# allentran/golds-rl-gym

Measured on AMD Instinct MI355X. Metric: env-steps/sec (whole node), 32k parallel Swarm-v0 envs, 20-step PAAC rollout, higher is better.
Workload: dtype f32; 1 GPU; Swarm-v0 84x84, 32768 envs per GPU, T=20 PAAC update, conv policy of train_paac_conv.py (BASELINE configs[2]); envs_per_gpu=32768, envs_total=32768, rollout_steps=20, policy=conv, train=True, swarm_math=exact, env_state_dtype=f64, streams=4, gradient_exchange=none

## Files before the change

golds-rl-gym_amd/csrc/api.hip:

```cpp
#include <string.h>

#include <algorithm>
#include <mutex>
#include <set>
#include <cmath>

#include "common.h"
#include "rollout_dev.h"

static thread_local std::string g_create_error;
static std::mutex g_live_mutex;
static std::set<const grl_handle *> g_live_handles;

namespace grl {
bool grl_handle_alive(const grl_handle *h) {
    std::lock_guard<std::mutex> lk(g_live_mutex);
    return g_live_handles.count(h) != 0;
}
void grl_sync_for_destroy(grl_handle *h) {
    if (grl_handle_alive(h)) {
        hipSetDevice(h->cfg.device_id);
        if (h->stream) hipStreamSynchronize(h->stream);
    } else {
        hipDeviceSynchronize();
// ... 47 lines not shown
            case GRL_FLD_RESET_XA: fi = {h->sw.rxa, 8, 20, false}; return h->sw.rxa != nullptr;
            case GRL_FLD_RESET_PNOISE: fi = {h->sw.rpnoise, 8, 160, false}; return h->sw.rpnoise != nullptr;
            case GRL_FLD_RESET_ANOISE: fi = {h->sw.ranoise, 8, 20, false}; return h->sw.ranoise != nullptr;
            default: return false;
        }
    }
    if (kind == GRL_ENV_SOLOW) {
        switch (f) {
            case GRL_FLD_SOLOW_K: fi = {h->so.k, 4, 1, false}; return true;
            case GRL_FLD_SOLOW_Z: fi = {h->so.z, 4, (size_t)h->so.P, true}; return true;
            case GRL_FLD_SOLOW_Z0: fi = {h->so.z0, 4, (size_t)h->so.P, true}; return true;
            case GRL_FLD_SOLOW_E: fi = {h->so.e, 4, (size_t)h->so.Q, true}; return true;
            case GRL_FLD_SOLOW_TAPE: fi = {h->so.tape, 4, (size_t)h->cfg.solow_tape_len, true}; return true;
            case GRL_FLD_SOLOW_TAPE_POS: fi = {h->so.tape_pos, 4, 1, false}; return true;
            case GRL_FLD_NHIST: fi = {h->so.nhist, 4, 1, false}; return true;
            default: return false;
        }
    }
    if (kind == GRL_ENV_TRADE) {
        size_t n = h->cfg.n_assets;
        switch (f) {
            case GRL_FLD_TRADE_CASH: fi = {h->tr.cash, 8, 1, false}; return true;
            case GRL_FLD_TRADE_ASSETS: fi = {h->tr.assets, 8, 1, false}; return true;
            case GRL_FLD_TRADE_QUANTITY: fi = {h->tr.q, 8, n, true}; return true;
            case GRL_FLD_TRADE_PRICES: fi = {h->tr.p, 8, n, true}; return true;
            case GRL_FLD_TRADE_NORMALS: fi = {h->tr.normals, 4, n, true}; return true;
            case GRL_FLD_NHIST: fi = {h->tr.nhist, 4, 1, false}; return true;
            default: return false;
        }
    }
    if (kind == GRL_ENV_TICKER) {
        switch (f) {
            case GRL_FLD_TICKER_CASH: fi = {h->tk.cash, 8, 1, false}; return true;
            case GRL_FLD_TICKER_ASSETS: fi = {h->tk.assets, 8, 1, false}; return true;
            case GRL_FLD_TICKER_QUANTITY: fi = {h->tk.q, 8, 2, false}; return true;
            case GRL_FLD_TICKER_IDX: fi = {h->tk.idx, 4, 1, false}; return true;
            case GRL_FLD_TICKER_START: fi = {h->tk.start, 4, 1, false}; return true;
            case GRL_FLD_TICKER_START0: fi = {h->tk.start0, 4, 1, false}; return true;
            case GRL_FLD_NHIST: fi = {h->tk.nhist, 4, 1, false}; return true;
            default: return false;
        }
    }
    return false;
}

static int action_cols(const grl_handle *h) {
    switch (h->cfg.env_kind) {
        case GRL_ENV_SWARM: return N_AGENTS * 2;
        case GRL_ENV_SOLOW: return 1;
        case GRL_ENV_TICKER: return 4;
        default: return h->cfg.n_assets;
    }
}

__global__ void episodes_account_kernel(const float *__restrict__ reward, const uint8_t *__restrict__ done, int env_base, int E,
                                        double *__restrict__ total, int32_t *__restrict__ len, int64_t *__restrict__ steps,
                                        grl_episode_record *__restrict__ rec, int32_t *__restrict__ count, int cap) {
    const int e = env_base + blockIdx.x * blockDim.x + threadIdx.x;
    const bool active = e < E;
    episodes_account_env(active, e, active ? reward[e] : 0.f, active && done[e] != 0, total, len, steps, rec, count, cap);
}

int episodes_launch_account(grl_handle *h, int env_base, int count) {
    if (!h->ep_total) return GRL_OK;
    if (count < 0) count = h->E - env_base;
    hipLaunchKernelGGL(episodes_account_kernel, dim3((count + 255) / 256), dim3(256), 0, h->stream, h->reward, h->done, env_base,
                       env_base + count, h->ep_total, h->ep_len, h->ep_steps, h->ep_rec, h->ep_count, h->ep_capacity);
    GRL_HIP(h, hipGetLastError());
    return GRL_OK;
}

static int reset_list(grl_handle *h, const int32_t *list_dev, const int32_t *count_dev, int max_count) {
    switch (h->cfg.env_kind) {
        case GRL_ENV_SWARM: return swarm_launch_reset(h, list_dev, count_dev, max_count);
        case GRL_ENV_SOLOW: return solow_launch_reset(h, list_dev, count_dev, max_count, true);
        case GRL_ENV_TICKER: return ticker_launch_reset(h, list_dev, count_dev, max_count);
        default: return trade_launch_reset(h, list_dev, count_dev, max_count);
    }
}

}

using namespace grl;

extern "C" {

int grl_abi_version(void) { return GRL_ABI_VERSION; }

int grl_config_default(int32_t env_kind, grl_config *cfg) {
    if (!cfg || env_kind < 0 || env_kind > GRL_ENV_TICKER) return GRL_E_INVALID;
    memset(cfg, 0, sizeof(*cfg));
    cfg->struct_size = (int32_t)sizeof(grl_config);
    cfg->env_kind = env_kind;
    cfg->num_envs = 32;
    cfg->max_episode_steps = env_kind == GRL_ENV_SWARM ? 128 : 1024;
    if (env_kind == GRL_ENV_TICKER) cfg->max_episode_steps = 1023;
    cfg->grid_size = 84;
    cfg->n_assets = 2;
    cfg->solow_p = 1; cfg->solow_q = 1;
    cfg->solow_tape_len = 2048;
    cfg->rnn_length = 5;
    cfg->seed = 1692;
    cfg->solow_sigma = 0.1; cfg->solow_delta = 0.02;
    cfg->trade_std_p = 0.05;
    cfg->trade_starting_balance = 10.0;
    return GRL_OK;
}

int grl_create(const grl_config *cfg, grl_handle **out) {
    if (!cfg || !out) return fail(nullptr, GRL_E_INVALID, "grl_create: null argument");
    *out = nullptr;
    if (cfg->struct_size != (int32_t)sizeof(grl_config)) return fail(nullptr, GRL_E_INVALID, "grl_create: grl_config size mismatch (ABI drift)");
    if (cfg->env_kind < 0 || cfg->env_kind > GRL_ENV_TICKER) return fail(nullptr, GRL_E_INVALID, "grl_create: unknown env_kind");
    if (cfg->env_kind == GRL_ENV_TICKER && (cfg->n_assets != 2 || cfg->rnn_length < 1 || cfg->rnn_length > 32))
        return fail(nullptr, GRL_E_INVALID, "grl_create: the Ticker table has two price columns (n_assets must be 2) and rnn_length must be in 1..32");
    if (cfg->env_kind == GRL_ENV_TICKER && (cfg->max_episode_steps < 0 || cfg->max_episode_steps > 1023))
        return fail(nullptr, GRL_E_INVALID, "grl_create: Ticker episodes live inside a 1024-row window: max_episode_steps must be in 0..1023 (0: no cap, stepping past the window is an error as in the reference)");
    if (cfg->num_envs <= 0) return fail(nullptr, GRL_E_INVALID, "grl_create: num_envs must be positive");
    if (cfg->env_kind == GRL_ENV_SWARM && (cfg->grid_size < 2 || cfg->grid_size > 254)) return fail(nullptr, GRL_E_INVALID, "grl_create: grid_size must be in 2..254");
    if (cfg->env_kind == GRL_ENV_TRADE && (cfg->n_assets < 1 || cfg->n_assets > 64)) return fail(nullptr, GRL_E_INVALID, "grl_create: n_assets must be in 1..64");
    if (cfg->env_kind == GRL_ENV_TRADE && !(cfg->trade_starting_balance > 0.0 && cfg->trade_starting_balance < 1e300))
        return fail(nullptr, GRL_E_INVALID, "grl_create: trade_starting_balance must be a positive finite number (the observation takes log(cash + 1e-4))");
    if (cfg->env_kind == GRL_ENV_SOLOW) {
        if (cfg->solow_p < 1 || cfg->solow_p > 8) return fail(nullptr, GRL_E_INVALID, "grl_create: solow_p must be in 1..8 (p=0 cannot reset in the reference either: fed_env.py:250 indexes an empty z)");
        if (cfg->solow_q < 0 || cfg->solow_q > 8) return fail(nullptr, GRL_E_INVALID, "grl_create: solow_q must be in 0..8");
        if (cfg->solow_tape_len < 2 || (cfg->solow_tape_len & 1)) return fail(nullptr, GRL_E_INVALID, "grl_create: solow_tape_len must be even and >= 2");
        if (cfg->rnn_length < 1 || cfg->rnn_length > 16) return fail(nullptr, GRL_E_INVALID, "grl_create: rnn_length must be in 1..16");
    }
    if (cfg->env_kind == GRL_ENV_TRADE && (cfg->rnn_length < 1 || cfg->rnn_length > 32))
        return fail(nullptr, GRL_E_INVALID, "grl_create: rnn_length must be in 1..32");
    int ndev = 0;
    hipError_t e = hipGetDeviceCount(&ndev);
    if (e != hipSuccess || ndev <= 0)
        return fail(nullptr, GRL_E_NO_DEVICE, std::string("grl_create: no HIP device available (") + (e != hipSuccess ? hipGetErrorString(e) : "count=0") + "); this library has no CPU path");
    if (cfg->device_id < 0 || cfg->device_id >= ndev) return fail(nullptr, GRL_E_NO_DEVICE, "grl_create: device_id out of range");
    hipDeviceProp_t prop;
    if ((e = hipGetDeviceProperties(&prop, cfg->device_id)) != hipSuccess) return fail(nullptr, GRL_E_HIP, std::string("hipGetDeviceProperties: ") + hipGetErrorString(e));
    if (strncmp(prop.gcnArchName, "gfx950", 6) != 0)
        return fail(nullptr, GRL_E_NO_DEVICE, std::string("grl_create: device is ") + prop.gcnArchName + ", this library is built for gfx950 (MI355X) only");
    if ((e = hipSetDevice(cfg->device_id)) != hipSuccess) return fail(nullptr, GRL_E_HIP, std::string("hipSetDevice: ") + hipGetErrorString(e));

    grl_handle *h = new grl_handle();
    {
        std::lock_guard<std::mutex> lk(g_live_mutex);
        g_live_handles.insert(h);
    }
    h->cfg = *cfg;
    h->E = cfg->num_envs;
    h->step_in_flight = false;
    h->prof_on = false; h->prof_used = 0;
    h->ep_total = nullptr; h->ep_len = nullptr; h->ep_steps = nullptr; h->ep_rec = nullptr; h->ep_count = nullptr; h->ep_capacity = 0;
    h->stream = nullptr; h->ev0 = nullptr; h->ev1 = nullptr;
    h->sw = {}; h->so = {}; h->tr = {}; h->tk = {};
    int rc = GRL_OK;
    auto bail = [&](int code) {
        g_create_error = h->err;
        grl_destroy(h);
        return code;
    };
    if ((e = hipStreamCreateWithFlags(&h->stream, hipStreamNonBlocking)) != hipSuccess) return bail(hip_fail(h, e, "hipStreamCreate"));
    if ((e = hipEventCreate(&h->ev0)) != hipSuccess || (e = hipEventCreate(&h->ev1)) != hipSuccess) return bail(hip_fail(h, e, "hipEventCreate"));
    size_t E = h->E;
    auto dm = [&](void **p, size_t bytes) -> int {
        hipError_t ee = hipMalloc(p, bytes);
        if (ee != hipSuccess) return hip_fail(h, ee, "hipMalloc");
        h->allocs.push_back(*p);
        ee = hipMemsetAsync(*p, 0, bytes, h->stream);
        return ee == hipSuccess ? GRL_OK : hip_fail(h, ee, "hipMemsetAsync");
    };
    h->actions_elems = E * action_cols(h);
    if ((rc = dm((void **)&h->elapsed, E * 4)) || (rc = dm((void **)&h->episode, E * 4)) || (rc = dm((void **)&h->reward, E * 4)) ||
        (rc = dm((void **)&h->done, E)) || (rc = dm((void **)&h->done_list, E * 4)) || (rc = dm((void **)&h->done_count, 16 * 4)) ||
        (rc = dm((void **)&h->err_flag, 4)) || (rc = dm((void **)&h->actions, h->actions_elems * 4)))
        return bail(rc);
    switch (cfg->env_kind) {
        case GRL_ENV_SWARM: rc = swarm_alloc(h); break;
        case GRL_ENV_SOLOW: rc = solow_alloc(h); break;
        case GRL_ENV_TICKER: rc = ticker_alloc(h); break;
        default: rc = trade_alloc(h); break;
    }
    if (rc) return bail(rc);
    if ((e = hipStreamSynchronize(h->stream)) != hipSuccess) return bail(hip_fail(h, e, "hipStreamSynchronize"));
    *out = h;
    return GRL_OK;
}

int grl_destroy(grl_handle *h) {
    if (!h) return GRL_OK;
    hipSetDevice(h->cfg.device_id);
    if (h->stream) hipStreamSynchronize(h->stream);
    for (void *p : h->allocs) hipFree(p);
    for (void *p : h->user_allocs) hipFree(p);
    for (hipEvent_t ev : h->prof_ev) hipEventDestroy(ev);
    if (h->ev0) hipEventDestroy(h->ev0);
    if (h->ev1) hipEventDestroy(h->ev1);
    if (h->stream) hipStreamDestroy(h->stream);
    {
        std::lock_guard<std::mutex> lk(g_live_mutex);
        g_live_handles.erase(h);
    }
    delete h;
    return GRL_OK;
}

const char *grl_last_error(const grl_handle *h) { return h ? h->err.c_str() : g_create_error.c_str(); }

int grl_reset(grl_handle *h, const int32_t *env_idx, int32_t n) {
    if (!h) return GRL_E_INVALID;
    hipSetDevice(h->cfg.device_id);
    int32_t cnt;
    if (env_idx == nullptr) {
        cnt = h->E;
        int rc = launch_iota(h, h->done_list, h->E);
        if (rc) return rc;
    } else {
        if (n < 0 || n > h->E) return fail(h, GRL_E_INVALID, "grl_reset: n out of range");
        for (int i = 0; i < n; ++i)
            if (env_idx[i] < 0 || env_idx[i] >= h->E) return fail(h, GRL_E_INVALID, "grl_reset: env index out of range");
        cnt = n;
        GRL_HIP(h, hipMemcpyAsync(h->done_list, env_idx, (size_t)n * 4, hipMemcpyHostToDevice, h->stream));
    }
    GRL_HIP(h, hipMemcpyAsync(h->done_count, &cnt, 4, hipMemcpyHostToDevice, h->stream));
    GRL_HIP(h, hipStreamSynchronize(h->stream));
    if (cnt > 0) {
        int rc = reset_list(h, h->done_list, h->done_count, cnt);
        if (rc) return rc;
    }
    GRL_HIP(h, hipStreamSynchronize(h->stream));
    return GRL_OK;
}

int grl_swarm_reset_injected(grl_handle *h, const double *x0, const double *xa0, const double *random_actions,
                             const double *agent_noise, const double *particle_noise) {
    if (!h || h->cfg.env_kind != GRL_ENV_SWARM) return fail(h, GRL_E_INVALID, "grl_swarm_reset_injected: not a Swarm handle");
    if (!x0 || !xa0 || !random_actions || !agent_noise || !particle_noise) return fail(h, GRL_E_INVALID, "grl_swarm_reset_injected: null argument");
    hipSetDevice(h->cfg.device_id);
    return swarm_reset_injected(h, x0, xa0, random_actions, agent_noise, particle_noise);
}

int grl_ticker_set_table(grl_handle *h, const double *rows, int32_t nrows) {
    if (!h || h->cfg.env_kind != GRL_ENV_TICKER) return fail(h, GRL_E_INVALID, "grl_ticker_set_table: not a Ticker handle");
    if (!rows) return fail(h, GRL_E_INVALID, "grl_ticker_set_table: null argument");
    hipSetDevice(h->cfg.device_id);
    return ticker_set_table(h, rows, nrows);
}

static int copy_field(grl_handle *h, int32_t field, void *host, size_t bytes, bool to_device) {
    if (!h || !host) return fail(h, GRL_E_INVALID, "grl_set/get_state: null argument");
    hipSetDevice(h->cfg.device_id);
    FieldInfo fi;
    if (!field_info(h, field, fi)) return fail(h, GRL_E_INVALID, "grl_set/get_state: field not valid for this env kind/config");
    size_t E = h->E, total = E * fi.inner * fi.elem;
    if (bytes != total) return fail(h, GRL_E_SIZE, "grl_set/get_state: host buffer is " + std::to_string(bytes) + " bytes, field needs " + std::to_string(total));
    GRL_HIP(h, hipStreamSynchronize(h->stream));
    if (!fi.feature_major || fi.inner == 1) {
        if (to_device) GRL_HIP(h, hipMemcpy(fi.dev, host, total, hipMemcpyHostToDevice));
        else GRL_HIP(h, hipMemcpy(host, fi.dev, total, hipMemcpyDeviceToHost));
        return GRL_OK;
    }
    auto transpose = [&](auto *hp, auto &tmp) -> int {
        if (to_device) {
            for (size_t e = 0; e < E; ++e)
                for (size_t i = 0; i < fi.inner; ++i) tmp[i * E + e] = hp[e * fi.inner + i];
            GRL_HIP(h, hipMemcpy(fi.dev, tmp.data(), total, hipMemcpyHostToDevice));
        } else {
            GRL_HIP(h, hipMemcpy(tmp.data(), fi.dev, total, hipMemcpyDeviceToHost));
            for (size_t e = 0; e < E; ++e)
                for (size_t i = 0; i < fi.inner; ++i) hp[e * fi.inner + i] = tmp[i * E + e];
        }
        return GRL_OK;
    };
    if (fi.elem == 8) {
        std::vector<uint64_t> tmp(E * fi.inner);
        return transpose((uint64_t *)host, tmp);
    }
    std::vector<uint32_t> tmp(E * fi.inner);
    return transpose((uint32_t *)host, tmp);
}

int grl_set_state(grl_handle *h, int32_t field, const void *host, size_t bytes) { return copy_field(h, field, (void *)host, bytes, true); }
int grl_get_state(grl_handle *h, int32_t field, void *host, size_t bytes) { return copy_field(h, field, host, bytes, false); }

int grl_step_device(grl_handle *h, const float *actions_dev) {
    if (!h || !actions_dev) return fail(h, GRL_E_INVALID, "grl_step_device: null argument");
    hipSetDevice(h->cfg.device_id);
    int rc;
    switch (h->cfg.env_kind) {
        case GRL_ENV_SWARM: rc = swarm_launch_step(h, actions_dev); break;
        case GRL_ENV_SOLOW: rc = solow_launch_step(h, actions_dev); break;
        case GRL_ENV_TICKER: rc = ticker_launch_step(h, actions_dev); break;
        default: rc = trade_launch_step(h, actions_dev); break;
    }
    if (rc == GRL_OK) rc = episodes_launch_account(h);
    if (rc == GRL_OK) h->step_in_flight = true;
    return rc;
}

int grl_step_async(grl_handle *h, const float *actions_host) {
    if (!h || !actions_host) return fail(h, GRL_E_INVALID, "grl_step_async: null argument");
    hipSetDevice(h->cfg.device_id);
    GRL_HIP(h, hipMemcpyAsync(h->actions, actions_host, h->actions_elems * 4, hipMemcpyHostToDevice, h->stream));
    return grl_step_device(h, h->actions);
}

int grl_swarm_step_f64(grl_handle *h, const double *actions_host) {
    if (!h || !actions_host) return fail(h, GRL_E_INVALID, "grl_swarm_step_f64: null argument");
// ... 369 lines not shown
```

golds-rl-gym_amd/csrc/common.h:

```cpp
#pragma once
#include <hip/hip_runtime.h>
#include <stdint.h>
#include <string>
#include <vector>

#include "../../include/goldsrl.h"

namespace grl {

constexpr int N_LOCUSTS = 80;
constexpr int N_AGENTS = 10;
constexpr int N_POINTS = 90;
constexpr int N_BURN_IN = 10;
constexpr int SWARM_EPB = 4;
constexpr int SWARM_TPB = SWARM_EPB * N_LOCUSTS;

enum : uint32_t {
    RS_SWARM_X0 = 0, RS_SWARM_XA0 = 1, RS_SWARM_RANDACT = 2, RS_SWARM_ANOISE = 3, RS_SWARM_PNOISE = 4,
    RS_SOLOW_Z0 = 8, RS_SOLOW_TAPE = 9, RS_TRADE_PRICE = 12, RS_TICKER_START = 16, RS_USER = 64
};

struct SwarmState {
    double *x, *xa, *pnoise, *anoise;
    double *rx, *rxa, *rpnoise, *ranoise;
    double *reward64;
    double *act64;
    uint8_t *lbins, *abins, *pos;
};

struct SolowState {
    float *k, *z, *e, *z0;
    float *tape;
    int32_t *tape_pos, *nhist;
    float *obs_raw, *obs, *history;
    float rho_z[8], rho_e[8];
    int P, Q;
};

struct TradeState {
    double *cash, *assets, *q, *p;
    float *normals;
    uint32_t *nstep;
    int32_t *nhist;
    float *obs_raw, *obs;
    double std_e;
    double start;
};

struct TickerState {
    double *cash, *assets, *q;
    double *reward64;
    int32_t *idx, *start, *start0;
    int32_t *nhist;
    float *obs_raw, *obs;
    const double *table;
    int rows;
};

}

struct grl_handle {
    grl_config cfg;
    int E;
    hipStream_t stream;
    hipEvent_t ev0, ev1;
    std::string err;
    bool step_in_flight;
    int32_t *elapsed, *episode;
    float *reward;
    uint8_t *done;
    int32_t *done_list, *done_count;
    int32_t *err_flag;
    float *actions;
    size_t actions_elems;
    grl::SwarmState sw;
    grl::SolowState so;
    grl::TradeState tr;
    grl::TickerState tk;
    std::vector<void *> allocs;
    std::vector<void *> user_allocs;
    double *ep_total;
    int32_t *ep_len;
    int64_t *ep_steps;
    grl_episode_record *ep_rec;
    int32_t *ep_count;
    int32_t ep_capacity;
    bool prof_on;
    std::vector<hipEvent_t> prof_ev;
    size_t prof_used;
};

namespace grl {
int fail(grl_handle *h, int code, const std::string &msg);
bool grl_handle_alive(const grl_handle *h);
void grl_sync_for_destroy(grl_handle *h);
void prof_begin(grl_handle *h);
void prof_end(grl_handle *h);
int hip_fail(grl_handle *h, hipError_t e, const char *what);
#define GRL_HIP(h, call)                                        \
    do {                                                        \
        hipError_t _e = (call);                                 \
        if (_e != hipSuccess) return grl::hip_fail(h, _e, #call); \
    } while (0)

int episodes_launch_account(grl_handle *h, int env_base = 0, int count = -1);
int swarm_alloc(grl_handle *h);
int swarm_launch_step(grl_handle *h, const float *actions_dev, const double *actions64_dev = nullptr, int no_wind = 0);
int swarm_launch_step_range(grl_handle *h, const float *actions_dev, int env_base, int count, int slot, bool counter_zeroed = false);
int swarm_launch_reset(grl_handle *h, const int32_t *list_dev, const int32_t *count_dev, int max_count);
int swarm_launch_observe(grl_handle *h);
int swarm_reset_injected(grl_handle *h, const double *x0, const double *xa0, const double *ra,
                         const double *an, const double *pn);
int swarm_materialize(grl_handle *h, int first, int count, float *out_dev);
int solow_alloc(grl_handle *h);
int solow_launch_step(grl_handle *h, const float *actions_dev);
int solow_launch_reset(grl_handle *h, const int32_t *list_dev, const int32_t *count_dev, int max_count, bool advance_episode);
int solow_launch_observe(grl_handle *h);
int trade_alloc(grl_handle *h);
int trade_launch_step(grl_handle *h, const float *actions_dev);
int trade_launch_reset(grl_handle *h, const int32_t *list_dev, const int32_t *count_dev, int max_count);
int trade_launch_observe(grl_handle *h);
int ticker_alloc(grl_handle *h);
int ticker_set_table(grl_handle *h, const double *rows_host, int nrows);
int ticker_launch_step(grl_handle *h, const float *actions_dev);
int ticker_launch_reset(grl_handle *h, const int32_t *list_dev, const int32_t *count_dev, int max_count);
int ticker_launch_observe(grl_handle *h);
int launch_returns(grl_handle *h, const float *r, const float *v, const float *mask, const float *boot, int T, int B,
                   float gamma, float lam, float scale, float clip_lo, float clip_hi, float *y, float *adv);
int launch_transform(grl_handle *h, int kind, float *actions_dev, int rows, int cols);
int launch_randn(grl_handle *h, float *dst, size_t n, uint32_t stream, uint64_t counter);
int launch_iota(grl_handle *h, int32_t *dst, int n);
}
```

golds-rl-gym_amd/csrc/swarm.hip:

```cpp
#include "common.h"
#include "rng.h"

namespace grl {

struct SwarmParams {
    double *x, *xa, *pnoise, *anoise;
    const double *rx, *rxa, *rpn, *ran;
    const double *inj_x0, *inj_xa0, *inj_ra, *inj_an, *inj_pn;
    const float *actions;
    const double *actions64;
    int32_t *elapsed, *episode;
    float *reward;
    double *reward64;
    uint8_t *done, *lbins, *abins, *pos;
    int32_t *done_list, *done_count;
    const int32_t *reset_list, *reset_count;
    int E, grid, max_steps;
    int env_base;
    uint32_t flags, env_off;
    uint64_t seed;
    int no_wind;
};

constexpr int LDS_STRIDE = 97;

struct SwarmLds {
    double2 p[SWARM_EPB][LDS_STRIDE];
    double en[SWARM_EPB][N_LOCUSTS];
    double meanx[SWARM_EPB];
    double rew[SWARM_EPB];
    int dflag[SWARM_EPB];
};

constexpr double DT = 0.05, NOISE = 0.0001, WIND = 1.0, GRAV = -1.0, FATT = 0.5, LATT = 10.0;

__device__ __forceinline__ void cutoff(double &y, double &vx, double &vy) {
    if (y <= 0) {
        y = 0;
        vx = 0;
        if (vy <= 0) vy = 0;
    }
}

__device__ __forceinline__ void x_update(double &x, double &y, double vx, double vy, double nx, double ny) {
    cutoff(y, vx, vy);
    x = x + (DT * vx + NOISE * nx);
    y = y + (DT * vy + NOISE * ny);
    if (y <= 0) y = 0;
}

__device__ __forceinline__ void x_update_f32v(double &x, double &y, float vx, float vy, double nx, double ny) {
    if (y <= 0) {
        y = 0;
        vx = 0;
        if (vy <= 0) vy = 0;
    }
    x = x + ((double)(0.05f * vx) + NOISE * nx);
    y = y + ((double)(0.05f * vy) + NOISE * ny);
    if (y <= 0) y = 0;
}

template <bool FAST>
__device__ __forceinline__ void pair_term(double sx, double sy, double xj, double yj, double &t0, double &t1) {
    double dx = sx - xj, dy = sy - yj;
    double d = sqrt(dx * dx + dy * dy);
    if (FAST) {
        double t = exp(d * -0.1);
        double t2 = t * t, t4 = t2 * t2, t5 = t4 * t, t10 = t5 * t5;
        double w = (FATT * t - t10) / (d + 0.000001);
        t0 = w * dx;
        t1 = w * dy;
    } else {
        double s = FATT * exp(-d / LATT) - exp(-d);
        double den = d + 0.000001;
        t0 = s * dx / den;
        t1 = s * dy / den;
    }
}

template <bool FAST>
__device__ __forceinline__ void locust_velocity(const double2 *src, double xj, double yj, double &vx, double &vy) {
    double a0[8], a1[8];
#pragma unroll
    for (int k = 0; k < 8; ++k) pair_term<FAST>(src[k].x, src[k].y, xj, yj, a0[k], a1[k]);
    for (int i = 8; i < N_LOCUSTS; i += 8) {
#pragma unroll
        for (int k = 0; k < 8; ++k) {
            double t0, t1;
            pair_term<FAST>(src[i + k].x, src[i + k].y, xj, yj, t0, t1);
            a0[k] += t0;
            a1[k] += t1;
        }
    }
    double ll0 = ((a0[0] + a0[1]) + (a0[2] + a0[3])) + ((a0[4] + a0[5]) + (a0[6] + a0[7]));
    double ll1 = ((a1[0] + a1[1]) + (a1[2] + a1[3])) + ((a1[4] + a1[5]) + (a1[6] + a1[7]));
#pragma unroll
    for (int k = 0; k < 8; ++k) pair_term<FAST>(src[N_LOCUSTS + k].x, src[N_LOCUSTS + k].y, xj, yj, a0[k], a1[k]);
    double al0 = ((a0[0] + a0[1]) + (a0[2] + a0[3])) + ((a0[4] + a0[5]) + (a0[6] + a0[7]));
    double al1 = ((a1[0] + a1[1]) + (a1[2] + a1[3])) + ((a1[4] + a1[5]) + (a1[6] + a1[7]));
#pragma unroll
    for (int k = 8; k < N_AGENTS; ++k) {
        double t0, t1;
        pair_term<FAST>(src[N_LOCUSTS + k].x, src[N_LOCUSTS + k].y, xj, yj, t0, t1);
        al0 += t0;
        al1 += t1;
    }
    vx = (WIND + ll0) + al0;
    vy = (GRAV + ll1) + al1;
}

template <bool FAST>
__device__ __forceinline__ void block_step(SwarmLds &L, int tid, int el, int j, double &xj, double &yj, double actx,
                                           double acty, double anx, double any, double pnx, double pny, bool act32 = false,
                                           bool wind = true) {
    if (tid < SWARM_EPB * N_AGENTS) {
        int ea = tid / N_AGENTS, a = tid - ea * N_AGENTS;
        double2 q = L.p[ea][N_LOCUSTS + a];
        if (act32) x_update_f32v(q.x, q.y, wind ? (float)actx + 1.0f : (float)actx, (float)acty, anx, any);
        else x_update(q.x, q.y, wind ? actx + WIND : actx, acty, anx, any);
        L.p[ea][N_LOCUSTS + a] = q;
    }
    L.p[el][j] = make_double2(xj, yj);
    __syncthreads();
    double vx, vy;
    locust_velocity<FAST>(L.p[el], xj, yj, vx, vy);
    L.en[el][j] = vx * vx + vy * vy;
    x_update(xj, yj, vx, vy, pnx, pny);
    __syncthreads();
    L.p[el][j] = make_double2(xj, yj);
    if (j == 0) {
        const double *e = L.en[el];
        double r[8];
#pragma unroll
        for (int k = 0; k < 8; ++k) r[k] = e[k];
        for (int i = 8; i < N_LOCUSTS; i += 8) {
#pragma unroll
            for (int k = 0; k < 8; ++k) r[k] += e[i + k];
        }
        double s = ((r[0] + r[1]) + (r[2] + r[3])) + ((r[4] + r[5]) + (r[6] + r[7]));
        L.rew[el] = -(s / (double)N_LOCUSTS);
    }
    __syncthreads();
}

__device__ __forceinline__ double edge_at(int k, double lo, double hi, double step, int G) {
    return (k >= G) ? hi : ((double)k * step + lo);
}
__device__ __forceinline__ int count_edges_le(double v, double lo, double hi, double step, int G) {
    if (!(v >= lo)) return 0;
    if (v >= hi) return G + 1;
    double gf = floor((v - lo) / step);
    int g = (gf > (double)G) ? G : (int)gf;
    if (g < 0) g = 0;
    for (int it = 0; it < 4 && g < G && edge_at(g + 1, lo, hi, step, G) <= v; ++it) ++g;
    for (int it = 0; it < 4 && g > 0 && edge_at(g, lo, hi, step, G) > v; ++it) --g;
    return g + 1;
}

enum { MODE_STEP = 0, MODE_OBSERVE = 1, MODE_RESET = 2 };

template <int MODE, bool FAST>
__global__ __launch_bounds__(SWARM_TPB, MODE == 0 ? 5 : 1) void swarm_kernel(SwarmParams P) {
    __shared__ SwarmLds L;
    __shared__ int env_of[SWARM_EPB];
    const int tid = threadIdx.x;
    const int el = tid / N_LOCUSTS, j = tid - el * N_LOCUSTS;

    if (MODE == MODE_RESET) {
        int cnt = *P.reset_count;
        if ((int)blockIdx.x * SWARM_EPB >= cnt) return;
        if (tid < SWARM_EPB) {
            int li = blockIdx.x * SWARM_EPB + tid;
            env_of[tid] = li < cnt ? P.reset_list[li] : -1;
        }
    } else {
        if (tid < SWARM_EPB) {
            int e = P.env_base + blockIdx.x * SWARM_EPB + tid;
            env_of[tid] = e < P.E ? e : -1;
        }
    }
    __syncthreads();
    const int env = env_of[el];
    const bool active = env >= 0;
    const int ea = tid / N_AGENTS, a = tid - ea * N_AGENTS;
    const bool agent_lane = tid < SWARM_EPB * N_AGENTS;
    const int aenv = agent_lane ? env_of[ea] : -1;
    const bool aactive = aenv >= 0;

    double xj = 0.5, yj = 0.5;
    if (MODE == MODE_STEP || MODE == MODE_OBSERVE) {
        if (active) {
            double2 q = reinterpret_cast<const double2 *>(P.x)[(size_t)env * N_LOCUSTS + j];
            xj = q.x; yj = q.y;
        }
        if (agent_lane) {
            double2 q = make_double2(0.5, 0.5);
            if (aactive) q = reinterpret_cast<const double2 *>(P.xa)[(size_t)aenv * N_AGENTS + a];
            L.p[ea][N_LOCUSTS + a] = q;
        }
    }

    if (MODE == MODE_STEP) {
        double actx = 0, acty = 0, anx = 0, any = 0, pnx = 0, pny = 0;
        if (active) {
            double2 n = reinterpret_cast<const double2 *>(P.pnoise)[(size_t)env * N_LOCUSTS + j];
            pnx = n.x; pny = n.y;
        }
        if (aactive) {
            if (P.actions64) {
                double2 act = reinterpret_cast<const double2 *>(P.actions64)[(size_t)aenv * N_AGENTS + a];
                actx = act.x; acty = act.y;
            } else {
                float2 act = reinterpret_cast<const float2 *>(P.actions)[(size_t)aenv * N_AGENTS + a];
                actx = (double)act.x; acty = (double)act.y;
            }
            double2 n = reinterpret_cast<const double2 *>(P.anoise)[(size_t)aenv * N_AGENTS + a];
            anx = n.x; any = n.y;
        }
        block_step<FAST>(L, tid, el, j, xj, yj, actx, acty, anx, any, pnx, pny, P.actions64 == nullptr, P.no_wind == 0);
        if (active) reinterpret_cast<double2 *>(P.x)[(size_t)env * N_LOCUSTS + j] = make_double2(xj, yj);
        if (aactive) reinterpret_cast<double2 *>(P.xa)[(size_t)aenv * N_AGENTS + a] = L.p[ea][N_LOCUSTS + a];
        if (active && j == 0) {
            double r = L.rew[el];
            int el_new = P.elapsed[env] + 1;
            bool d = (r >= 0) || (P.max_steps > 0 && el_new >= P.max_steps);
            P.elapsed[env] = el_new;
            P.reward64[env] = r;
            P.reward[env] = (float)r;
            P.done[env] = d ? 1 : 0;
            L.dflag[el] = d ? env : -1;
        } else if (j == 0) {
            L.dflag[el] = -1;
        }
        __syncthreads();
        if (tid == 0) {
            int n = 0;
#pragma unroll
            for (int e = 0; e < SWARM_EPB; ++e) n += L.dflag[e] >= 0 ? 1 : 0;
            if (n) {
                int slot = atomicAdd(P.done_count, n);
#pragma unroll
                for (int e = 0; e < SWARM_EPB; ++e)
                    if (L.dflag[e] >= 0) P.done_list[slot++] = L.dflag[e];
            }
        }
    }

    if (MODE == MODE_RESET) {
        const uint32_t genv = active ? (uint32_t)env + P.env_off : 0u;
        const uint32_t gaenv = aactive ? (uint32_t)aenv + P.env_off : 0u;
        const uint32_t ep = (active && !(P.flags & GRL_F_RESEED_EACH_RESET)) ? (uint32_t)P.episode[env] : 0u;
        const uint32_t aep = (aactive && !(P.flags & GRL_F_RESEED_EACH_RESET)) ? (uint32_t)P.episode[aenv] : 0u;
        double pn10x = 0, pn10y = 0, an10x = 0, an10y = 0;
        if (P.flags & GRL_F_RESET_FROM_SNAPSHOT) {
            if (active) {
                double2 q = reinterpret_cast<const double2 *>(P.rx)[(size_t)env * N_LOCUSTS + j];
                xj = q.x; yj = q.y;
                double2 n = reinterpret_cast<const double2 *>(P.rpn)[(size_t)env * N_LOCUSTS + j];
                pn10x = n.x; pn10y = n.y;
            }
            if (agent_lane) {
                double2 q = make_double2(0.5, 0.5);
                if (aactive) {
                    q = reinterpret_cast<const double2 *>(P.rxa)[(size_t)aenv * N_AGENTS + a];
                    double2 n = reinterpret_cast<const double2 *>(P.ran)[(size_t)aenv * N_AGENTS + a];
                    an10x = n.x; an10y = n.y;
                }
                L.p[ea][N_LOCUSTS + a] = q;
            }
            L.p[el][j] = make_double2(xj, yj);
            __syncthreads();
        } else {
            const bool inj = P.inj_x0 != nullptr;
            if (inj) {
                if (active) {
                    double2 q = reinterpret_cast<const double2 *>(P.inj_x0)[(size_t)env * N_LOCUSTS + j];
                    xj = q.x; yj = q.y;
                }
            } else {
                u01_pair(rng_block(P.seed, genv, ep, RS_SWARM_X0, j), xj, yj);
            }
            if (agent_lane) {
                double2 q = make_double2(0.5, 0.5);
                if (inj) {
                    if (aactive) q = reinterpret_cast<const double2 *>(P.inj_xa0)[(size_t)aenv * N_AGENTS + a];
                } else {
                    u01_pair(rng_block(P.seed, gaenv, aep, RS_SWARM_XA0, a), q.x, q.y);
                }
                L.p[ea][N_LOCUSTS + a] = q;
            }
            for (int t = 0; t <= N_BURN_IN; ++t) {
                double actx = 0, acty = 0, anx = 0, any = 0, pnx = 0, pny = 0;
                if (inj) {
                    if (active) {
                        double2 n = reinterpret_cast<const double2 *>(P.inj_pn)[((size_t)env * (N_BURN_IN + 1) + t) * N_LOCUSTS + j];
                        pnx = n.x; pny = n.y;
                    }
                    if (aactive) {
                        double2 n = reinterpret_cast<const double2 *>(P.inj_an)[((size_t)aenv * (N_BURN_IN + 1) + t) * N_AGENTS + a];
                        anx = n.x; any = n.y;
                        if (t < N_BURN_IN) {
                            double2 r = reinterpret_cast<const double2 *>(P.inj_ra)[((size_t)aenv * N_BURN_IN + t) * N_AGENTS + a];
                            actx = r.x; acty = r.y;
                        }
                    }
                } else {
                    normal_pair(rng_block(P.seed, genv, ep, RS_SWARM_PNOISE, t * N_LOCUSTS + j), pnx, pny);
                    if (agent_lane) {
                        normal_pair(rng_block(P.seed, gaenv, aep, RS_SWARM_ANOISE, t * N_AGENTS + a), anx, any);
                        if (t < N_BURN_IN) normal_pair(rng_block(P.seed, gaenv, aep, RS_SWARM_RANDACT, t * N_AGENTS + a), actx, acty);
                    }
                }
                if (t == N_BURN_IN) {
                    pn10x = pnx; pn10y = pny; an10x = anx; an10y = any;
                    break;
                }
                block_step<FAST>(L, tid, el, j, xj, yj, actx, acty, anx, any, pnx, pny);
            }
        }
        if (active) {
            reinterpret_cast<double2 *>(P.x)[(size_t)env * N_LOCUSTS + j] = make_double2(xj, yj);
            reinterpret_cast<double2 *>(P.pnoise)[(size_t)env * N_LOCUSTS + j] = make_double2(pn10x, pn10y);
            if (j == 0) {
                P.elapsed[env] = 0;
                P.episode[env] = P.episode[env] + 1;
            }
        }
        if (aactive) {
            reinterpret_cast<double2 *>(P.xa)[(size_t)aenv * N_AGENTS + a] = L.p[ea][N_LOCUSTS + a];
            reinterpret_cast<double2 *>(P.anoise)[(size_t)aenv * N_AGENTS + a] = make_double2(an10x, an10y);
        }
    }

    if (MODE == MODE_OBSERVE) {
        L.p[el][j] = make_double2(xj, yj);
        __syncthreads();
    }

    if (P.flags & GRL_F_SWARM_NO_OBSERVE) return;
    if (j == 0) {
        double s = L.p[el][0].x;
        for (int i = 1; i < N_POINTS; ++i) s += L.p[el][i].x;
        L.meanx[el] = s / (double)N_POINTS;
    }
    __syncthreads();
    const int G = P.grid;
    const double ylo = 0.0, yhi = 6.0;
    const double ystep = (yhi - ylo) / (double)G;
    {
        double m = L.meanx[el];
        double lo = m - 1.5, hi = m + 1.5;
        double step = (hi - lo) / (double)G;
        int cx = count_edges_le(xj, lo, hi, step, G);
        int cy = count_edges_le(yj, ylo, yhi, ystep, G);
        int bx = (xj == hi) ? G - 1 : cx - 1;
        int by = (yj == yhi) ? G - 1 : cy - 1;
        bool in = bx >= 0 && bx < G && by >= 0 && by < G;
        if (active) reinterpret_cast<uint16_t *>(P.lbins)[(size_t)env * N_LOCUSTS + j] = in ? (uint16_t)(bx | (by << 8)) : (uint16_t)0xFFFF;
    }
    if (aactive) {
        double2 q = L.p[ea][N_LOCUSTS + a];
        double m = L.meanx[ea];
        double lo = m - 1.5, hi = m + 1.5;
        double step = (hi - lo) / (double)G;
        int cx = count_edges_le(q.x, lo, hi, step, G);
        int cy = count_edges_le(q.y, ylo, yhi, ystep, G);
        int bx = (q.x == hi) ? G - 1 : cx - 1;
        int by = (q.y == yhi) ? G - 1 : cy - 1;
        bool in = bx >= 0 && bx < G && by >= 0 && by < G;
        reinterpret_cast<uint16_t *>(P.abins)[(size_t)aenv * N_AGENTS + a] = in ? (uint16_t)(bx | (by << 8)) : (uint16_t)0xFFFF;
        int px = cx >= G ? G - 1 : cx;
        int py = cy >= G ? G - 1 : cy;
        reinterpret_cast<uint16_t *>(P.pos)[(size_t)aenv * N_AGENTS + a] = (uint16_t)(px | (py << 8));
    }
}

__global__ void swarm_materialize_kernel(const uint8_t *lbins, const uint8_t *abins, const uint8_t *pos, int first, int G,
                                         float *out) {
    extern __shared__ unsigned int cnt[];
    const int env = first + blockIdx.x;
    const int GG = G * G;
    for (int i = threadIdx.x; i < 2 * GG; i += blockDim.x) cnt[i] = 0;
    __syncthreads();
    if (threadIdx.x < N_LOCUSTS) {
        int bx = lbins[((size_t)env * N_LOCUSTS + threadIdx.x) * 2], by = lbins[((size_t)env * N_LOCUSTS + threadIdx.x) * 2 + 1];
        if (bx != 255) atomicAdd(&cnt[bx * G + by], 1u);
    } else if (threadIdx.x < N_POINTS) {
        int a = threadIdx.x - N_LOCUSTS;
        int bx = abins[((size_t)env * N_AGENTS + a) * 2], by = abins[((size_t)env * N_AGENTS + a) * 2 + 1];
        if (bx != 255) atomicAdd(&cnt[GG + bx * G + by], 1u);
    }
    __syncthreads();
    float *o = out + (size_t)blockIdx.x * N_AGENTS * GG * 3;
    for (int a = 0; a < N_AGENTS; ++a) {
        int px = pos[((size_t)env * N_AGENTS + a) * 2], py = pos[((size_t)env * N_AGENTS + a) * 2 + 1];
        int hot = px * G + py;
        for (int i = threadIdx.x; i < GG * 3; i += blockDim.x) {
            int pix = i / 3, c = i - pix * 3;
            float v;
            if (c == 0) v = (float)((double)cnt[pix] / 80.0);
            else if (c == 1) v = (float)((double)cnt[GG + pix] / 10.0);
            else v = (pix == hot) ? 1.0f : 0.0f;
            o[(size_t)a * GG * 3 + i] = v;
        }
    }
}

static SwarmParams make_params(grl_handle *h) {
    SwarmParams P{};
    P.x = h->sw.x; P.xa = h->sw.xa; P.pnoise = h->sw.pnoise; P.anoise = h->sw.anoise;
    P.rx = h->sw.rx; P.rxa = h->sw.rxa; P.rpn = h->sw.rpnoise; P.ran = h->sw.ranoise;
    P.elapsed = h->elapsed; P.episode = h->episode; P.reward = h->reward; P.reward64 = h->sw.reward64;
    P.done = h->done; P.lbins = h->sw.lbins; P.abins = h->sw.abins; P.pos = h->sw.pos;
    P.done_list = h->done_list; P.done_count = h->done_count;
    P.E = h->E; P.grid = h->cfg.grid_size; P.max_steps = h->cfg.max_episode_steps;
    P.flags = h->cfg.flags; P.env_off = (uint32_t)h->cfg.env_id_offset; P.seed = h->cfg.seed;
    return P;
}

template <typename T>
static int dmalloc(grl_handle *h, T **p, size_t n) {
    GRL_HIP(h, hipMalloc((void **)p, n * sizeof(T)));
    h->allocs.push_back(*p);
    GRL_HIP(h, hipMemsetAsync(*p, 0, n * sizeof(T), h->stream));
    return GRL_OK;
}

int swarm_alloc(grl_handle *h) {
    size_t E = h->E;
    int rc;
    if ((rc = dmalloc(h, &h->sw.x, E * N_LOCUSTS * 2))) return rc;
    if ((rc = dmalloc(h, &h->sw.xa, E * N_AGENTS * 2))) return rc;
    if ((rc = dmalloc(h, &h->sw.pnoise, E * N_LOCUSTS * 2))) return rc;
    if ((rc = dmalloc(h, &h->sw.anoise, E * N_AGENTS * 2))) return rc;
    if ((rc = dmalloc(h, &h->sw.reward64, E))) return rc;
    if ((rc = dmalloc(h, &h->sw.lbins, E * N_LOCUSTS * 2))) return rc;
    if ((rc = dmalloc(h, &h->sw.abins, E * N_AGENTS * 2))) return rc;
    if ((rc = dmalloc(h, &h->sw.pos, E * N_AGENTS * 2))) return rc;
    if (h->cfg.flags & GRL_F_RESET_FROM_SNAPSHOT) {
        if ((rc = dmalloc(h, &h->sw.rx, E * N_LOCUSTS * 2))) return rc;
        if ((rc = dmalloc(h, &h->sw.rxa, E * N_AGENTS * 2))) return rc;
        if ((rc = dmalloc(h, &h->sw.rpnoise, E * N_LOCUSTS * 2))) return rc;
        if ((rc = dmalloc(h, &h->sw.ranoise, E * N_AGENTS * 2))) return rc;
    }
    return GRL_OK;
}

static inline int nblocks(int n) { return (n + SWARM_EPB - 1) / SWARM_EPB; }

int swarm_launch_step(grl_handle *h, const float *actions_dev, const double *actions64_dev, int no_wind) {
    SwarmParams P = make_params(h);
    P.actions = actions_dev;
    P.actions64 = actions64_dev;
    P.no_wind = no_wind;
    GRL_HIP(h, hipMemsetAsync(h->done_count, 0, sizeof(int32_t), h->stream));
    prof_begin(h);
    if (h->cfg.flags & GRL_F_SWARM_FAST_MATH)
        hipLaunchKernelGGL((swarm_kernel<MODE_STEP, true>), dim3(nblocks(h->E)), dim3(SWARM_TPB), 0, h->stream, P);
    else
        hipLaunchKernelGGL((swarm_kernel<MODE_STEP, false>), dim3(nblocks(h->E)), dim3(SWARM_TPB), 0, h->stream, P);
    prof_end(h);
    GRL_HIP(h, hipGetLastError());
    return swarm_launch_reset(h, h->done_list, h->done_count, h->E);
}

int swarm_launch_step_range(grl_handle *h, const float *actions_dev, int env_base, int count, int slot, bool counter_zeroed) {
    SwarmParams P = make_params(h);
    P.actions = actions_dev;
    P.actions64 = nullptr;
    P.env_base = env_base;
    P.E = env_base + count;
    P.done_list = h->done_list + env_base;
    P.done_count = h->done_count + slot;
    if (!counter_zeroed) GRL_HIP(h, hipMemsetAsync(P.done_count, 0, sizeof(int32_t), h->stream));
    if (h->cfg.flags & GRL_F_SWARM_FAST_MATH)
        hipLaunchKernelGGL((swarm_kernel<MODE_STEP, true>), dim3(nblocks(count)), dim3(SWARM_TPB), 0, h->stream, P);
    else
        hipLaunchKernelGGL((swarm_kernel<MODE_STEP, false>), dim3(nblocks(count)), dim3(SWARM_TPB), 0, h->stream, P);
    GRL_HIP(h, hipGetLastError());
    return swarm_launch_reset(h, P.done_list, P.done_count, count);
}

int swarm_launch_reset(grl_handle *h, const int32_t *list_dev, const int32_t *count_dev, int max_count) {
    SwarmParams P = make_params(h);
    P.reset_list = list_dev;
    P.reset_count = count_dev;
    if (h->cfg.flags & GRL_F_SWARM_FAST_MATH)
        hipLaunchKernelGGL((swarm_kernel<MODE_RESET, true>), dim3(nblocks(max_count)), dim3(SWARM_TPB), 0, h->stream, P);
    else
        hipLaunchKernelGGL((swarm_kernel<MODE_RESET, false>), dim3(nblocks(max_count)), dim3(SWARM_TPB), 0, h->stream, P);
    GRL_HIP(h, hipGetLastError());
    return GRL_OK;
}

int swarm_launch_observe(grl_handle *h) {
    SwarmParams P = make_params(h);
    P.flags &= ~GRL_F_SWARM_NO_OBSERVE;
    hipLaunchKernelGGL((swarm_kernel<MODE_OBSERVE, false>), dim3(nblocks(h->E)), dim3(SWARM_TPB), 0, h->stream, P);
    GRL_HIP(h, hipGetLastError());
    return GRL_OK;
}

int swarm_reset_injected(grl_handle *h, const double *x0, const double *xa0, const double *ra, const double *an,
                         const double *pn) {
    size_t E = h->E;
    size_t n_x0 = E * N_LOCUSTS * 2, n_xa0 = E * N_AGENTS * 2, n_ra = E * N_BURN_IN * N_AGENTS * 2;
    size_t n_an = E * (N_BURN_IN + 1) * N_AGENTS * 2, n_pn = E * (N_BURN_IN + 1) * N_LOCUSTS * 2;
    double *buf = nullptr;
    GRL_HIP(h, hipMalloc((void **)&buf, (n_x0 + n_xa0 + n_ra + n_an + n_pn) * sizeof(double)));
    double *d_x0 = buf, *d_xa0 = d_x0 + n_x0, *d_ra = d_xa0 + n_xa0, *d_an = d_ra + n_ra, *d_pn = d_an + n_an;
    hipError_t e = hipSuccess;
    if (e == hipSuccess) e = hipMemcpyAsync(d_x0, x0, n_x0 * 8, hipMemcpyHostToDevice, h->stream);
    if (e == hipSuccess) e = hipMemcpyAsync(d_xa0, xa0, n_xa0 * 8, hipMemcpyHostToDevice, h->stream);
    if (e == hipSuccess) e = hipMemcpyAsync(d_ra, ra, n_ra * 8, hipMemcpyHostToDevice, h->stream);
    if (e == hipSuccess) e = hipMemcpyAsync(d_an, an, n_an * 8, hipMemcpyHostToDevice, h->stream);
    if (e == hipSuccess) e = hipMemcpyAsync(d_pn, pn, n_pn * 8, hipMemcpyHostToDevice, h->stream);
    int rc = GRL_OK;
    if (e == hipSuccess) {
        rc = launch_iota(h, h->done_list, h->E);
        int32_t cnt = h->E;
        if (rc == GRL_OK) e = hipMemcpyAsync(h->done_count, &cnt, sizeof(cnt), hipMemcpyHostToDevice, h->stream);
        if (rc == GRL_OK && e == hipSuccess) {
            e = hipStreamSynchronize(h->stream);
            SwarmParams P = make_params(h);
            P.flags &= ~(GRL_F_RESET_FROM_SNAPSHOT);
            P.reset_list = h->done_list; P.reset_count = h->done_count;
            P.inj_x0 = d_x0; P.inj_xa0 = d_xa0; P.inj_ra = d_ra; P.inj_an = d_an; P.inj_pn = d_pn;
            if (h->cfg.flags & GRL_F_SWARM_FAST_MATH)
                hipLaunchKernelGGL((swarm_kernel<MODE_RESET, true>), dim3(nblocks(h->E)), dim3(SWARM_TPB), 0, h->stream, P);
            else
                hipLaunchKernelGGL((swarm_kernel<MODE_RESET, false>), dim3(nblocks(h->E)), dim3(SWARM_TPB), 0, h->stream, P);
            if (e == hipSuccess) e = hipGetLastError();
            if (e == hipSuccess) e = hipStreamSynchronize(h->stream);
        }
    }
    hipFree(buf);
    if (rc != GRL_OK) return rc;
    if (e != hipSuccess) return hip_fail(h, e, "swarm_reset_injected");
    return GRL_OK;
}

int swarm_materialize(grl_handle *h, int first, int count, float *out_dev) {
    int G = h->cfg.grid_size;
    size_t lds = (size_t)2 * G * G * sizeof(unsigned int);
    hipLaunchKernelGGL(swarm_materialize_kernel, dim3(count), dim3(256), lds, h->stream, h->sw.lbins, h->sw.abins,
                       h->sw.pos, first, G, out_dev);
    GRL_HIP(h, hipGetLastError());
    return GRL_OK;
}

}
```

Measured before the change: 2.216 million env-steps/s.

## Compute locust pair interactions once per pair using antisymmetry via LDS tile ring

Replaces the all-pairs locust velocity loop, where each thread evaluates interactions with all 80 locusts, with a compile-time pair schedule. Each unordered pair is computed once and stored, with its sign-flipped counterpart, in 8x8 tiles of a shared-memory ring; threads then accumulate their row from those tiles. This roughly halves the double-precision pair_term work, but adds many __syncthreads barriers, LDS traffic and larger shared memory, which may reduce occupancy. The old direct path stays available through the GRL_SWARM_PAIRS=direct environment variable.

```diff
diff --git a/golds-rl-gym_amd/csrc/api.hip b/golds-rl-gym_amd/csrc/api.hip
--- a/golds-rl-gym_amd/csrc/api.hip
+++ b/golds-rl-gym_amd/csrc/api.hip
@@ -223,6 +223,7 @@
     h->ep_total = nullptr; h->ep_len = nullptr; h->ep_steps = nullptr; h->ep_rec = nullptr; h->ep_count = nullptr; h->ep_capacity = 0;
     h->stream = nullptr; h->ev0 = nullptr; h->ev1 = nullptr;
     h->sw = {}; h->so = {}; h->tr = {}; h->tk = {};
+    if (const char *sp = getenv("GRL_SWARM_PAIRS")) h->sw.pairs_direct = strcmp(sp, "direct") == 0;
     int rc = GRL_OK;
     auto bail = [&](int code) {
         g_create_error = h->err;
diff --git a/golds-rl-gym_amd/csrc/common.h b/golds-rl-gym_amd/csrc/common.h
--- a/golds-rl-gym_amd/csrc/common.h
+++ b/golds-rl-gym_amd/csrc/common.h
@@ -26,6 +26,7 @@
     double *reward64;
     double *act64;
     uint8_t *lbins, *abins, *pos;
+    bool pairs_direct;
 };
 
 struct SolowState {
diff --git a/golds-rl-gym_amd/csrc/swarm.hip b/golds-rl-gym_amd/csrc/swarm.hip
--- a/golds-rl-gym_amd/csrc/swarm.hip
+++ b/golds-rl-gym_amd/csrc/swarm.hip
@@ -24,9 +24,66 @@
 
 constexpr int LDS_STRIDE = 97;
 
-struct SwarmLds {
+constexpr int PAIR_BLK = N_LOCUSTS / 8;
+constexpr int N_TAU = 2 * PAIR_BLK - 1;
+constexpr int N_PAIRS = N_LOCUSTS * (N_LOCUSTS - 1) / 2;
+constexpr int PAIR_U = 2;
+constexpr int SLOT_PAIRS = PAIR_U * N_LOCUSTS;
+constexpr int N_SLOTS = (N_PAIRS + SLOT_PAIRS - 1) / SLOT_PAIRS;
+constexpr int RING_TILES = 8;
+constexpr uint32_t PW_DIAG = 1u << 20, PW_SELF_LO = 1u << 21, PW_SELF_HI = 1u << 22;
+static_assert(N_LOCUSTS % 8 == 0, "pair tiles are 8 x 8");
+
+struct PairSched {
+    uint32_t e[N_SLOTS * SLOT_PAIRS];
+    int tile0[N_TAU];
+    int slot[N_TAU];
+    bool ok;
+};
+
+constexpr PairSched make_pair_sched() {
+    PairSched S{};
+    int n = 0, g = 0;
+    int first_slot[64] = {}, tile_tau[64] = {};
+    for (int tau = 0; tau < N_TAU; ++tau) {
+        S.tile0[tau] = g;
+        for (int a = tau >= PAIR_BLK ? tau - (PAIR_BLK - 1) : 0; a <= tau / 2; ++a, ++g) {
+            const int b = tau - a;
+            first_slot[g] = n / SLOT_PAIRS;
+            tile_tau[g] = tau;
+            for (int p = 0; p < 8; ++p)
+                for (int q = 0; q < 8; ++q) {
+                    if (a == b && p >= q) continue;
+                    uint32_t w = (uint32_t)(8 * a + p) | (uint32_t)(8 * b + q) << 8 | (uint32_t)(g % RING_TILES) << 16;
+                    if (a == b) w |= PW_DIAG | (q == p + 1 ? PW_SELF_LO : 0u) | (p == 0 && q == 7 ? PW_SELF_HI : 0u);
+                    S.e[n++] = w;
+                }
+        }
+        S.slot[tau] = (n - 1) / SLOT_PAIRS;
+    }
+    S.ok = n == N_PAIRS && g <= 64;
+    for (int k = 0; n < N_SLOTS * SLOT_PAIRS; ++n, ++k) S.e[n] = S.e[N_PAIRS - 1 - k % 8];
+    for (int t = RING_TILES; t < g; ++t)
+        if (first_slot[t] <= S.slot[tile_tau[t - RING_TILES]]) S.ok = false;
+    return S;
+}
+static_assert(make_pair_sched().ok, "pair ring too small for the slot schedule");
+__constant__ PairSched kPairSched = make_pair_sched();
+
+template <bool PAIRS> struct SwarmLds;
+template <> struct SwarmLds<false> {
     double2 p[SWARM_EPB][LDS_STRIDE];
     double en[SWARM_EPB][N_LOCUSTS];
+    double meanx[SWARM_EPB];
+    double rew[SWARM_EPB];
+    int dflag[SWARM_EPB];
+};
+template <> struct SwarmLds<true> {
+    double2 p[SWARM_EPB][LDS_STRIDE];
+    union {
+        double2 ring[SWARM_EPB][RING_TILES * 64];
+        double en[SWARM_EPB][N_LOCUSTS];
+    };
     double meanx[SWARM_EPB];
     double rew[SWARM_EPB];
     int dflag[SWARM_EPB];
@@ -79,6 +136,25 @@
 }
 
 template <bool FAST>
+__device__ __forceinline__ void agent_tail(const double2 *src, double xj, double yj, double ll0, double ll1, double &vx,
+                                           double &vy) {
+    double a0[8], a1[8];
+#pragma unroll
+    for (int k = 0; k < 8; ++k) pair_term<FAST>(src[N_LOCUSTS + k].x, src[N_LOCUSTS + k].y, xj, yj, a0[k], a1[k]);
+    double al0 = ((a0[0] + a0[1]) + (a0[2] + a0[3])) + ((a0[4] + a0[5]) + (a0[6] + a0[7]));
+    double al1 = ((a1[0] + a1[1]) + (a1[2] + a1[3])) + ((a1[4] + a1[5]) + (a1[6] + a1[7]));
+#pragma unroll
+    for (int k = 8; k < N_AGENTS; ++k) {
+        double t0, t1;
+        pair_term<FAST>(src[N_LOCUSTS + k].x, src[N_LOCUSTS + k].y, xj, yj, t0, t1);
+        al0 += t0;
+        al1 += t1;
+    }
+    vx = (WIND + ll0) + al0;
+    vy = (GRAV + ll1) + al1;
+}
+
+template <bool FAST>
 __device__ __forceinline__ void locust_velocity(const double2 *src, double xj, double yj, double &vx, double &vy) {
     double a0[8], a1[8];
 #pragma unroll
@@ -94,23 +170,80 @@
     }
     double ll0 = ((a0[0] + a0[1]) + (a0[2] + a0[3])) + ((a0[4] + a0[5]) + (a0[6] + a0[7]));
     double ll1 = ((a1[0] + a1[1]) + (a1[2] + a1[3])) + ((a1[4] + a1[5]) + (a1[6] + a1[7]));
-#pragma unroll
-    for (int k = 0; k < 8; ++k) pair_term<FAST>(src[N_LOCUSTS + k].x, src[N_LOCUSTS + k].y, xj, yj, a0[k], a1[k]);
-    double al0 = ((a0[0] + a0[1]) + (a0[2] + a0[3])) + ((a0[4] + a0[5]) + (a0[6] + a0[7]));
-    double al1 = ((a1[0] + a1[1]) + (a1[2] + a1[3])) + ((a1[4] + a1[5]) + (a1[6] + a1[7]));
-#pragma unroll
-    for (int k = 8; k < N_AGENTS; ++k) {
-        double t0, t1;
-        pair_term<FAST>(src[N_LOCUSTS + k].x, src[N_LOCUSTS + k].y, xj, yj, t0, t1);
-        al0 += t0;
-        al1 += t1;
-    }
-    vx = (WIND + ll0) + al0;
-    vy = (GRAV + ll1) + al1;
+    agent_tail<FAST>(src, xj, yj, ll0, ll1, vx, vy);
+}
+__device__ __forceinline__ double flip_sign(double v, uint32_t m) {
+    return __hiloint2double(__double2hiint(v) ^ (int)m, __double2loint(v));
+}
+
+template <bool FAST, int U>
+__device__ __forceinline__ void pair_slot(const double2 *src, double2 *ring, const uint32_t *w) {
+    double t0[U], t1[U];
+#pragma unroll
+    for (int u = 0; u < U; ++u) {
+        const int lo = w[u] & 127, hi = (w[u] >> 8) & 127;
+        pair_term<FAST>(src[lo].x, src[lo].y, src[hi].x, src[hi].y, t0[u], t1[u]);
+    }
+#pragma unroll
+    for (int u = 0; u < U; ++u) {
+        const uint32_t e = w[u];
+        const int lo = e & 7, hi = (e >> 8) & 7, at = lo * 8 + hi;
+        double2 *t = ring + ((e >> 16) & (RING_TILES - 1)) * 64;
+        const double2 v = make_double2(t0[u], t1[u]);
+        t[at] = v;
+        const bool diag = (e & PW_DIAG) != 0;
+        const uint32_t neg = diag ? 0x80000000u : 0u;
+        t[diag ? hi * 8 + lo : at] = make_double2(flip_sign(v.x, neg), flip_sign(v.y, neg));
+        const bool self = (e & (PW_SELF_LO | PW_SELF_HI)) != 0;
+        t[self ? ((e & PW_SELF_LO) ? lo : hi) * 9 : at] = self ? make_double2(-0.0, -0.0) : v;
+    }
 }
 
 template <bool FAST>
-__device__ __forceinline__ void block_step(SwarmLds &L, int tid, int el, int j, double &xj, double &yj, double actx,
+__device__ __forceinline__ void locust_velocity_pairs(const double2 *src, double2 *ring, int j, double xj, double yj,
+                                                      double &vx, double &vy) {
+    const int bj = j >> 3, cj = j & 7;
+    double a0[8], a1[8];
+#pragma unroll
+    for (int k = 0; k < 8; ++k) a0[k] = a1[k] = -0.0;
+    uint32_t w[PAIR_U];
+#pragma unroll
+    for (int u = 0; u < PAIR_U; ++u) w[u] = kPairSched.e[u * N_LOCUSTS + j];
+    int tau = 0;
+    for (int s = 0; s < N_SLOTS; ++s) {
+        uint32_t wn[PAIR_U];
+#pragma unroll
+        for (int u = 0; u < PAIR_U; ++u) wn[u] = s + 1 < N_SLOTS ? kPairSched.e[(s + 1) * SLOT_PAIRS + u * N_LOCUSTS + j] : 0u;
+        pair_slot<FAST, PAIR_U>(src, ring, w);
+        __syncthreads();
+        for (; tau < N_TAU && kPairSched.slot[tau] == s; ++tau) {
+            const int m = tau - bj;
+            if (m >= 0 && m < PAIR_BLK) {
+                const int amin = tau >= PAIR_BLK ? tau - (PAIR_BLK - 1) : 0;
+                const bool below = m <= bj;
+                const int tile = (kPairSched.tile0[tau] + (below ? m : bj) - amin) & (RING_TILES - 1);
+                const double2 *t = ring + tile * 64 + (below ? cj : cj * 8);
+                const int stride = below ? 8 : 1;
+                const uint32_t neg = below ? 0u : 0x80000000u;
+#pragma unroll
+                for (int k = 0; k < 8; ++k) {
+                    double2 v = t[k * stride];
+                    a0[k] += flip_sign(v.x, neg);
+                    a1[k] += flip_sign(v.y, neg);
+                }
+            }
+        }
+        __syncthreads();
+#pragma unroll
+        for (int u = 0; u < PAIR_U; ++u) w[u] = wn[u];
+    }
+    double ll0 = ((a0[0] + a0[1]) + (a0[2] + a0[3])) + ((a0[4] + a0[5]) + (a0[6] + a0[7]));
+    double ll1 = ((a1[0] + a1[1]) + (a1[2] + a1[3])) + ((a1[4] + a1[5]) + (a1[6] + a1[7]));
+    agent_tail<FAST>(src, xj, yj, ll0, ll1, vx, vy);
+}
+
+template <bool FAST, bool PAIRS>
+__device__ __forceinline__ void block_step(SwarmLds<PAIRS> &L, int tid, int el, int j, double &xj, double &yj, double actx,
                                            double acty, double anx, double any, double pnx, double pny, bool act32 = false,
                                            bool wind = true) {
     if (tid < SWARM_EPB * N_AGENTS) {
@@ -123,7 +256,11 @@
     L.p[el][j] = make_double2(xj, yj);
     __syncthreads();
     double vx, vy;
-    locust_velocity<FAST>(L.p[el], xj, yj, vx, vy);
+    if constexpr (PAIRS) {
+        locust_velocity_pairs<FAST>(L.p[el], L.ring[el], j, xj, yj, vx, vy);
+    } else {
+        locust_velocity<FAST>(L.p[el], xj, yj, vx, vy);
+    }
     L.en[el][j] = vx * vx + vy * vy;
     x_update(xj, yj, vx, vy, pnx, pny);
     __syncthreads();
@@ -159,9 +296,9 @@
 
 enum { MODE_STEP = 0, MODE_OBSERVE = 1, MODE_RESET = 2 };
 
-template <int MODE, bool FAST>
+template <int MODE, bool FAST, bool PAIRS>
 __global__ __launch_bounds__(SWARM_TPB, MODE == 0 ? 5 : 1) void swarm_kernel(SwarmParams P) {
-    __shared__ SwarmLds L;
+    __shared__ SwarmLds<PAIRS> L;
     __shared__ int env_of[SWARM_EPB];
     const int tid = threadIdx.x;
     const int el = tid / N_LOCUSTS, j = tid - el * N_LOCUSTS;
@@ -217,7 +354,7 @@
             double2 n = reinterpret_cast<const double2 *>(P.anoise)[(size_t)aenv * N_AGENTS + a];
             anx = n.x; any = n.y;
         }
-        block_step<FAST>(L, tid, el, j, xj, yj, actx, acty, anx, any, pnx, pny, P.actions64 == nullptr, P.no_wind == 0);
+        block_step<FAST, PAIRS>(L, tid, el, j, xj, yj, actx, acty, anx, any, pnx, pny, P.actions64 == nullptr, P.no_wind == 0);
         if (active) reinterpret_cast<double2 *>(P.x)[(size_t)env * N_LOCUSTS + j] = make_double2(xj, yj);
         if (aactive) reinterpret_cast<double2 *>(P.xa)[(size_t)aenv * N_AGENTS + a] = L.p[ea][N_LOCUSTS + a];
         if (active && j == 0) {
@@ -315,7 +452,7 @@
                     pn10x = pnx; pn10y = pny; an10x = anx; an10y = any;
                     break;
                 }
-                block_step<FAST>(L, tid, el, j, xj, yj, actx, acty, anx, any, pnx, pny);
+                block_step<FAST, PAIRS>(L, tid, el, j, xj, yj, actx, acty, anx, any, pnx, pny);
             }
         }
         if (active) {
@@ -448,6 +585,14 @@
 
 static inline int nblocks(int n) { return (n + SWARM_EPB - 1) / SWARM_EPB; }
 
+template <int MODE>
+static void launch_swarm(grl_handle *h, int blocks, const SwarmParams &P) {
+    const bool fast = (h->cfg.flags & GRL_F_SWARM_FAST_MATH) != 0, direct = h->sw.pairs_direct;
+    void (*k)(SwarmParams) = fast ? (direct ? swarm_kernel<MODE, true, false> : swarm_kernel<MODE, true, true>)
+                                  : (direct ? swarm_kernel<MODE, false, false> : swarm_kernel<MODE, false, true>);
+    hipLaunchKernelGGL(k, dim3(blocks), dim3(SWARM_TPB), 0, h->stream, P);
+}
+
 int swarm_launch_step(grl_handle *h, const float *actions_dev, const double *actions64_dev, int no_wind) {
     SwarmParams P = make_params(h);
     P.actions = actions_dev;
@@ -455,10 +600,7 @@
     P.no_wind = no_wind;
     GRL_HIP(h, hipMemsetAsync(h->done_count, 0, sizeof(int32_t), h->stream));
     prof_begin(h);
-    if (h->cfg.flags & GRL_F_SWARM_FAST_MATH)
-        hipLaunchKernelGGL((swarm_kernel<MODE_STEP, true>), dim3(nblocks(h->E)), dim3(SWARM_TPB), 0, h->stream, P);
-    else
-        hipLaunchKernelGGL((swarm_kernel<MODE_STEP, false>), dim3(nblocks(h->E)), dim3(SWARM_TPB), 0, h->stream, P);
+    launch_swarm<MODE_STEP>(h, nblocks(h->E), P);
     prof_end(h);
     GRL_HIP(h, hipGetLastError());
     return swarm_launch_reset(h, h->done_list, h->done_count, h->E);
@@ -473,10 +615,7 @@
     P.done_list = h->done_list + env_base;
     P.done_count = h->done_count + slot;
     if (!counter_zeroed) GRL_HIP(h, hipMemsetAsync(P.done_count, 0, sizeof(int32_t), h->stream));
-    if (h->cfg.flags & GRL_F_SWARM_FAST_MATH)
-        hipLaunchKernelGGL((swarm_kernel<MODE_STEP, true>), dim3(nblocks(count)), dim3(SWARM_TPB), 0, h->stream, P);
-    else
-        hipLaunchKernelGGL((swarm_kernel<MODE_STEP, false>), dim3(nblocks(count)), dim3(SWARM_TPB), 0, h->stream, P);
+    launch_swarm<MODE_STEP>(h, nblocks(count), P);
     GRL_HIP(h, hipGetLastError());
     return swarm_launch_reset(h, P.done_list, P.done_count, count);
 }
@@ -485,10 +624,7 @@
     SwarmParams P = make_params(h);
     P.reset_list = list_dev;
     P.reset_count = count_dev;
-    if (h->cfg.flags & GRL_F_SWARM_FAST_MATH)
-        hipLaunchKernelGGL((swarm_kernel<MODE_RESET, true>), dim3(nblocks(max_count)), dim3(SWARM_TPB), 0, h->stream, P);
-    else
-        hipLaunchKernelGGL((swarm_kernel<MODE_RESET, false>), dim3(nblocks(max_count)), dim3(SWARM_TPB), 0, h->stream, P);
+    launch_swarm<MODE_RESET>(h, nblocks(max_count), P);
     GRL_HIP(h, hipGetLastError());
     return GRL_OK;
 }
@@ -496,7 +632,7 @@
 int swarm_launch_observe(grl_handle *h) {
     SwarmParams P = make_params(h);
     P.flags &= ~GRL_F_SWARM_NO_OBSERVE;
-    hipLaunchKernelGGL((swarm_kernel<MODE_OBSERVE, false>), dim3(nblocks(h->E)), dim3(SWARM_TPB), 0, h->stream, P);
+    hipLaunchKernelGGL((swarm_kernel<MODE_OBSERVE, false, false>), dim3(nblocks(h->E)), dim3(SWARM_TPB), 0, h->stream, P);
     GRL_HIP(h, hipGetLastError());
     return GRL_OK;
 }
@@ -526,10 +662,7 @@
             P.flags &= ~(GRL_F_RESET_FROM_SNAPSHOT);
             P.reset_list = h->done_list; P.reset_count = h->done_count;
             P.inj_x0 = d_x0; P.inj_xa0 = d_xa0; P.inj_ra = d_ra; P.inj_an = d_an; P.inj_pn = d_pn;
-            if (h->cfg.flags & GRL_F_SWARM_FAST_MATH)
-                hipLaunchKernelGGL((swarm_kernel<MODE_RESET, true>), dim3(nblocks(h->E)), dim3(SWARM_TPB), 0, h->stream, P);
-            else
-                hipLaunchKernelGGL((swarm_kernel<MODE_RESET, false>), dim3(nblocks(h->E)), dim3(SWARM_TPB), 0, h->stream, P);
+            launch_swarm<MODE_RESET>(h, nblocks(h->E), P);
             if (e == hipSuccess) e = hipGetLastError();
             if (e == hipSuccess) e = hipStreamSynchronize(h->stream);
         }
```

Measured after the change: 2.202 million env-steps/s, median of 4. Within noise of the previous version (-0.6%).
